# deflect-ca/banjax

Hardware: AMD Instinct MI355X
Metric: log lines/sec matched+rate-limited (node) at 1k rules; HBM GB/s vs peak (higher is better)
Workload: dtype u8

## Files before the change

banjax_amd/_lib.py:

```python
from __future__ import annotations

import ctypes as C
import os

HERE = os.path.dirname(os.path.abspath(__file__))
LIB_PATH = os.environ.get("BJX_LIB_PATH") or os.path.join(HERE, "lib", "libbanjax_gpu.so")

OK = 0
ERR_REGEX, ERR_ARG, ERR_DEVICE, ERR_NOMEM, ERR_TOO_COMPLEX, ERR_CAPACITY, ERR_DECISION = -1, -2, -3, -4, -5, -6, -7
TAIL_STOPPED, ERR_IO = -8, -9
INPUT_DEVICE, COPY_RESULTS, EMIT_BANS, BAN_RECORDS_ONLY, TRIPS_COMPACT, RULE_STATS = 1, 2, 4, 8, 16, 32


class Str(C.Structure):
    _fields_ = [("ptr", C.c_char_p), ("len", C.c_size_t)]


class RuleSpec(C.Structure):
    _fields_ = [("name", Str), ("regex", Str), ("interval_ns", C.c_int64), ("hits_per_interval", C.c_int64),
                ("decision", C.c_int32), ("hosts_to_skip", C.POINTER(Str)), ("n_hosts_to_skip", C.c_size_t)]


class SiteRules(C.Structure):
    _fields_ = [("host", Str), ("rules", C.POINTER(RuleSpec)), ("n_rules", C.c_size_t)]
# ... 207 lines not shown
    L.bjx_finish_batch_trips.argtypes = [vp, vp, C.c_uint64, C.c_uint32, C.POINTER(BatchResult)]
    L.bjx_state_get.restype = C.c_int
    L.bjx_state_get.argtypes = [vp, C.c_char_p, sz, C.c_char_p, sz, C.POINTER(C.c_int64), C.POINTER(C.c_int64)]
    L.bjx_state_len.restype = C.c_int64
    L.bjx_state_len.argtypes = [vp]
    L.bjx_state_stats_get.restype = C.c_int
    L.bjx_state_stats_get.argtypes = [vp, C.c_void_p]
    L.bjx_state_clear.restype = C.c_int
    L.bjx_state_clear.argtypes = [vp]
    L.bjx_state_dump.restype = sz
    L.bjx_state_dump.argtypes = [vp, C.c_char_p, sz]
    L.bjx_debug_rule_match_host.restype = C.c_int
    L.bjx_debug_rule_match_host.argtypes = [vp, sz, C.c_char_p, sz]
    L.bjx_debug_regex_parse.restype = C.c_int
    L.bjx_debug_regex_parse.argtypes = [C.c_char_p, sz, C.c_char_p, sz]
    L.bjx_debug_rule_lead.restype = C.c_int
    L.bjx_debug_rule_lead.argtypes = [vp, sz]
    L.bjx_debug_rule_literal.restype = sz
    L.bjx_debug_rule_literal.argtypes = [vp, sz, C.c_char_p, sz]
    L.bjx_debug_ruleset_literals.restype = sz
    L.bjx_debug_ruleset_literals.argtypes = [vp]
    L.bjx_debug_phase_ms.restype = sz
    L.bjx_debug_phase_ms.argtypes = [vp, C.POINTER(C.c_double), sz]
    L.bjx_debug_kernel_ms.restype = sz
    L.bjx_debug_kernel_ms.argtypes = [vp, C.POINTER(C.c_double), sz]
    L.bjx_debug_scan_stats.restype = sz
    L.bjx_debug_scan_stats.argtypes = [vp, C.POINTER(C.c_uint64), sz]
    L.bjx_debug_set_claim_budget.restype = C.c_int
    L.bjx_debug_set_claim_budget.argtypes = [vp, C.c_uint64]
    L.bjx_debug_set_slot_cache.restype = C.c_int
# ... 113 lines not shown
```

banjax_amd/csrc/engine.hip:

```cpp
#include <hip/hip_runtime.h>
#include <hipcub/hipcub.hpp>

#include <algorithm>
#include <array>
#include <atomic>
#include <cstdio>
#include <cstdlib>
#include <cstring>
#include <map>
#include <set>
#include <tuple>
#include <memory>
#include <mutex>
#include <stdexcept>
#include <string>
#include <unordered_map>
#include <thread>
#include <vector>

#include "../../include/banjax_gpu.h"
#include "bjx_common.h"
#include "engine_types.h"
#include "allow_entry.h"
#include "regex_compiler.h"
#include "bans.h"
#include "snapshot.h"
#include "state_query.h"
#include "state_remove.h"
#include "state_nets.h"
#include "state_trim.h"

using namespace bjx;

namespace {

struct BjxError : std::runtime_error {
// ... 2083 lines not shown
}

__device__ __forceinline__ uint32_t lead_start_seek(const Bind &B, const DevRule &R, const Lines &L, const uint8_t *buf,
                                                    uint64_t n_buf, uint64_t j, uint32_t pos, uint64_t rs, uint32_t rl) {
  const uint32_t st0 = lead_start(B, L, j, pos, rs, rl);
  if ((R.lead & 3u) != 3u || st0 >= rl || B.cfirst || L.cand_meta[j].cnt <= (uint32_t)kCandSlots) return st0;
  const uint32_t back = R.lead_dist ? R.lead_dist + 3u : 0u;
  const uint64_t q = lead_seek(B, R, buf, n_buf, rs + st0 + (st0 ? back : 0u), rs + rl);
  const uint32_t o = (uint32_t)(q - rs);
  return o >= rl ? rl : (o > back && o - back > st0 ? o - back : st0);
}

constexpr uint32_t kDfaLdsEntries = 8192;
constexpr uint32_t kDfaAccelLds = 2048;

__device__ __forceinline__ uint32_t accel_mask(const uint4 v, uint32_t ac) {
  const uint32_t wv[4] = {v.x, v.y, v.z, v.w};
  const uint32_t ne = (ac >> 24) & 3u;
  uint32_t m = 0;
#pragma unroll
  for (int q = 0; q < 4; ++q) {
    uint32_t hb = wv[q] & 0x80808080u;
#pragma unroll
    for (uint32_t k = 0; k < 3; ++k) {
      if (k >= ne) break;
      const uint32_t y = wv[q] ^ (((ac >> (8 * k)) & 0xFFu) * 0x01010101u);
      hb |= ~(((y & 0x7F7F7F7Fu) + 0x7F7F7F7Fu) | y) & 0x80808080u;
    }
    m |= (((hb >> 7) & 1u) | ((hb >> 14) & 2u) | ((hb >> 21) & 4u) | ((hb >> 28) & 8u)) << (4 * q);
  }
  return m;
}

template <bool STAGED>
__device__ __forceinline__ bool dfa_text(const Bind &B, const DevRule &R, const uint16_t *tr, const uint8_t *ac,
                                         const uint32_t *acc, const uint8_t *__restrict__ buf, uint64_t n_buf, uint64_t t0,
                                         uint32_t len, uint32_t st0) {
  const uint32_t ncls = R.ncls;
  uint32_t st = st0;
  uint64_t a = t0 & ~15ull;
  const uint64_t end = t0 + len;
  uint32_t skip = (uint32_t)(t0 - a);
  auto load16 = [&](uint64_t p) -> uint4 {
    if (p + 16 <= n_buf) return *reinterpret_cast<const uint4 *>(buf + p);
    uint32_t w[4];
    for (int k = 0; k < 4; ++k) {
      uint32_t x = 0;
      for (int b = 0; b < 4; ++b) x |= (p + 4 * k + b < n_buf ? (uint32_t)buf[p + 4 * k + b] : 0u) << (8 * b);
      w[k] = x;
    }
    return make_uint4(w[0], w[1], w[2], w[3]);
  };
  uint4 v = a < end ? load16(a) : make_uint4(0, 0, 0, 0);
  while (a < end) {
    const uint32_t aw = acc ? acc[st] : 0u;
    if (aw >> 31) {
      for (;;) {
        uint32_t m = accel_mask(v, aw) & ~((1u << skip) - 1u);
        if (end - a < 16) m &= (1u << (uint32_t)(end - a)) - 1u;
        if (m) { skip = (uint32_t)__ffs(m) - 1; break; }
        a += 16;
        skip = 0;
        if (a >= end) return B.accept_end[R.ae_off + st] != 0;
        v = load16(a);
      }
    }
    const uint4 vn = a + 16 < end ? load16(a + 16) : make_uint4(0, 0, 0, 0);
    const uint32_t wv[4] = {v.x, v.y, v.z, v.w};
    const uint32_t lim = end - a < 16 ? (uint32_t)(end - a) : 16u;
#pragma unroll
    for (uint32_t k = 0; k < 16; ++k) {
      if (k < skip || k >= lim) continue;
      const uint32_t b = (wv[k >> 2] >> (8 * (k & 3))) & 0xFF;
      if (b >= 0x80) {
        const DevRule *Rp = &R;
        uint64_t i = a + k;
        while (i < end) {
          int w;
          const int32_t rune = decode_rune_hd(buf + i, (uint32_t)(end - i), &w);
          uint32_t c;
          if (rune < 0x80) c = ac[rune];
          else {
            const uint32_t *na = B.nonascii + 2 * Rp->na_off;
            uint32_t lo = 0, hi = Rp->n_na;
            while (hi - lo > 1) {
              const uint32_t m = (lo + hi) >> 1;
              if (na[2 * m] <= (uint32_t)rune) lo = m; else hi = m;
            }
            c = na[2 * lo + 1];
          }
          i += (uint32_t)w;
          st = tr[st * ncls + c];
          if (st <= 1) break;
        }
        return B.accept_end[R.ae_off + st] != 0;
      }
      st = tr[st * ncls + ac[b]];
      if (st <= 1) return st == kAccept;
    }
    skip = 0;
    a += 16;
    v = vn;
  }
  return B.accept_end[R.ae_off + st] != 0;
}

__device__ __forceinline__ uint32_t nl_mask16(const uint4 v) {
  return flag_mask16(nl_mask_word(v.x), nl_mask_word(v.y), nl_mask_word(v.z), nl_mask_word(v.w));
}
template <bool STAGED>
__device__ __forceinline__ bool dfa_line(const Bind &B, const DevRule &R, const uint16_t *tr, const uint8_t *ac,
                                         const uint32_t *acc, const uint8_t *__restrict__ buf, uint64_t n_buf, uint64_t t0,
                                         uint32_t st0) {
  const uint32_t ncls = R.ncls;
  uint32_t st = st0;
  uint64_t a = t0 & ~15ull;
  uint32_t skip = (uint32_t)(t0 - a);
  auto load16 = [&](uint64_t p) -> uint4 {
    if (p + 16 <= n_buf) return *reinterpret_cast<const uint4 *>(buf + p);
    uint32_t w[4];
    for (int k = 0; k < 4; ++k) {
      uint32_t x = 0;
      for (int b = 0; b < 4; ++b) x |= (p + 4 * k + b < n_buf ? (uint32_t)buf[p + 4 * k + b] : 0x0Au) << (8 * b);
      w[k] = x;
    }
    return make_uint4(w[0], w[1], w[2], w[3]);
  };
  uint4 v = load16(a);
  for (;;) {
    uint32_t nlm = nl_mask16(v) & ~((1u << skip) - 1u);
    const uint32_t aw = acc ? acc[st] : 0u;
    if ((aw >> 31) && !nlm) {
      for (;;) {
        const uint32_t m = accel_mask(v, aw) & ~((1u << skip) - 1u);
        if (m || nlm) {
          const uint32_t f = (uint32_t)__ffs(m | nlm) - 1;
          skip = f;
          break;
        }
        a += 16;
        skip = 0;
        v = load16(a);
        nlm = nl_mask16(v);
      }
    } else if (aw >> 31) {
      const uint32_t m = (accel_mask(v, aw) | nlm) & ~((1u << skip) - 1u);
      skip = (uint32_t)__ffs(m) - 1;
    }
    const uint32_t lim = nlm ? (uint32_t)__ffs(nlm) - 1 : 16u;
    const uint4 vn = lim == 16u ? load16(a + 16) : make_uint4(0, 0, 0, 0);
    const uint32_t wv[4] = {v.x, v.y, v.z, v.w};
#pragma unroll
    for (uint32_t k = 0; k < 16; ++k) {
      if (k < skip || k >= lim) continue;
      const uint32_t b = (wv[k >> 2] >> (8 * (k & 3))) & 0xFF;
      if (b >= 0x80) {
        uint64_t i = a + k, end = i;
        while (end < n_buf && buf[end] != '\n') ++end;
        while (i < end) {
          int w;
          const int32_t rune = decode_rune_hd(buf + i, (uint32_t)(end - i), &w);
          uint32_t c;
          if (rune < 0x80) c = ac[rune];
          else {
            const uint32_t *na = B.nonascii + 2 * R.na_off;
            uint32_t lo = 0, hi = R.n_na;
            while (hi - lo > 1) {
              const uint32_t m = (lo + hi) >> 1;
              if (na[2 * m] <= (uint32_t)rune) lo = m; else hi = m;
            }
            c = na[2 * lo + 1];
          }
          i += (uint32_t)w;
          st = tr[st * ncls + c];
          if (st <= 1) break;
        }
        return B.accept_end[R.ae_off + st] != 0;
      }
      st = tr[st * ncls + ac[b]];
      if (st <= 1) return st == kAccept;
    }
    if (lim < 16u) return B.accept_end[R.ae_off + st] != 0;
    skip = 0;
    a += 16;
    v = vn;
  }
}

__global__ __launch_bounds__(kBlock) void k_dfa(Bind B, const uint8_t *__restrict__ buf, uint64_t n_buf,
                                                const uint32_t *__restrict__ jkey, const uint32_t *__restrict__ jidx,
                                                const uint32_t *__restrict__ jline, const uint64_t *__restrict__ jrec, uint64_t n,
                                                Lines L) {
  extern __shared__ __attribute__((aligned(16))) uint8_t s_dfa[];
  uint16_t *s_tr = reinterpret_cast<uint16_t *>(s_dfa);
  uint32_t *s_acc = reinterpret_cast<uint32_t *>(s_dfa + ((B.dfa_tr * 2 + 15) & ~15u));
  uint8_t *s_ac = reinterpret_cast<uint8_t *>(s_acc + B.dfa_acc);
  const uint64_t t0 = (uint64_t)blockIdx.x * blockDim.x;
  if ((jkey[t0] & 0xFFFFFF) >= B.n_rules) return;
  const uint64_t t = t0 + threadIdx.x;
  const uint64_t tl = t0 + blockDim.x - 1 < n ? t0 + blockDim.x - 1 : n - 1;
  const uint32_t r0 = jkey[t0] & 0xFFFFFF;
  const DevRule R0 = B.rules[r0];
  const bool uniform = (jkey[tl] & 0xFFFFFF) == r0;
  const bool staged = uniform && (uint32_t)R0.ncls * R0.n_states <= B.dfa_tr;
  if (staged) {
    const uint16_t *g = B.trans + R0.trans_off;
    for (uint32_t i = threadIdx.x; i < (uint32_t)R0.ncls * R0.n_states; i += blockDim.x) s_tr[i] = g[i];
    if (threadIdx.x < 128) s_ac[threadIdx.x] = B.ascii_cls[(size_t)r0 * 128 + threadIdx.x];
    if (R0.n_states <= B.dfa_acc)
      for (uint32_t i = threadIdx.x; i < R0.n_states; i += blockDim.x) s_acc[i] = B.accel[R0.ae_off + i];
  }
  __syncthreads();
  if (t >= n) return;
  const uint32_t key = jkey[t];
  const uint32_t r = key & 0xFFFFFF, pos = key >> 24;
  if (r >= B.n_rules) return;
  const uint32_t slot = jidx[t];
  const uint64_t rec = jrec[slot];
  const uint64_t a = rec & kJobOffMask;
  bool m;
  if (staged) {
    const uint32_t *acc = R0.n_states <= B.dfa_acc ? s_acc : B.accel + R0.ae_off;
    m = dfa_line<true>(B, R0, s_tr, s_ac, acc, buf, n_buf, a, (rec & kJobSkipState) ? R0.skip_state : R0.start);
  } else {
    const DevRule R = B.rules[r];
    m = dfa_line<false>(B, R, B.trans + R.trans_off, B.ascii_cls + (size_t)r * 128, B.accel + R.ae_off, buf, n_buf, a,
                        (rec & kJobSkipState) ? R.skip_state : R.start);
  }
  if (!m) return;
  const uint64_t j = jline[slot];
  atomicOr(reinterpret_cast<unsigned long long *>(&L.mword(j, pos >> 6)), 1ull << (pos & 63));
  atomicAdd(reinterpret_cast<unsigned long long *>(L.counts + j), (1ull << 32) | ((rec & kJobNoCount) ? 0ull : 1ull));
}

__global__ __launch_bounds__(kBlock) void k_dfa_legacy(Bind B, const uint8_t *__restrict__ buf, uint64_t n_buf,
                                                       const uint64_t *__restrict__ nl, const uint32_t *__restrict__ jkey,
                                                       const uint32_t *__restrict__ jidx, const uint32_t *__restrict__ jline,
                                                       uint64_t n, Lines L) {
  __shared__ uint16_t s_tr[kDfaLdsEntries];
  __shared__ uint32_t s_acc[kDfaAccelLds];
  __shared__ uint8_t s_ac[128];
  const uint64_t t0 = (uint64_t)blockIdx.x * blockDim.x;
  const uint64_t t = t0 + threadIdx.x;
  const uint64_t tl = t0 + blockDim.x - 1 < n ? t0 + blockDim.x - 1 : n - 1;
  if ((jkey[tl] & 0xFFFFFF) < B.n_rules) return;
  const uint32_t k0 = jkey[t0] & 0xFFFFFF;
  const uint32_t r0 = k0 >= B.n_rules ? k0 - B.n_rules : k0;
  const DevRule R0 = B.rules[r0];
  const bool uniform = k0 >= B.n_rules && (jkey[tl] & 0xFFFFFF) == k0;
  if (uniform && (R0.flags & kRuleNfa)) return;
  const bool staged = uniform && (uint32_t)R0.ncls * R0.n_states <= kDfaLdsEntries;
  if (staged) {
    const uint16_t *g = B.trans + R0.trans_off;
    for (uint32_t i = threadIdx.x; i < (uint32_t)R0.ncls * R0.n_states; i += blockDim.x) s_tr[i] = g[i];
    if (threadIdx.x < 128) s_ac[threadIdx.x] = B.ascii_cls[(size_t)r0 * 128 + threadIdx.x];
    if (R0.n_states <= kDfaAccelLds)
      for (uint32_t i = threadIdx.x; i < R0.n_states; i += blockDim.x) s_acc[i] = B.accel[R0.ae_off + i];
  }
  __syncthreads();
  if (t >= n) return;
  const uint32_t key = jkey[t];
  const uint32_t rk = key & 0xFFFFFF, pos = key >> 24;
  if (rk < B.n_rules) return;
  const uint32_t r = rk - B.n_rules;
  const uint64_t j = jline[jidx[t]];
  const uint64_t s = j ? nl[j - 1] + 1 : 0;
  const uint64_t rs = s + L.rest_off[j];
  const uint32_t rl = (uint32_t)(nl[j] - rs);
  bool m;
  if (!staged && (B.rules[r].flags & kRuleNfa)) return;
  if ((staged ? R0.equiv : B.rules[r].equiv) && eq_certain(B, L, j, pos, rs)) {
    m = true;
  } else if (staged) {
    const uint32_t sk = R0.skip_len && R0.skip_len <= rl ? R0.skip_len : 0u;
    const uint32_t st0 = (R0.lead & 1u) ? lead_start_seek(B, R0, L, buf, n_buf, j, pos, rs, rl) : 0u;
    const uint32_t *acc = R0.n_states <= kDfaAccelLds ? s_acc : B.accel + R0.ae_off;
    m = st0 ? dfa_text<true>(B, R0, s_tr, s_ac, acc, buf, n_buf, rs + st0, rl - st0, R0.start)
            : dfa_text<true>(B, R0, s_tr, s_ac, acc, buf, n_buf, rs + sk, rl - sk, sk ? R0.skip_state : R0.start);
  } else {
    const DevRule R = B.rules[r];
    const uint32_t sk = R.skip_len && R.skip_len <= rl ? R.skip_len : 0u;
    const uint32_t st0 = (R.lead & 1u) ? lead_start_seek(B, R, L, buf, n_buf, j, pos, rs, rl) : 0u;
    const uint32_t *acc = B.accel + R.ae_off;
    if (st0) m = dfa_text<false>(B, R, B.trans + R.trans_off, B.ascii_cls + (size_t)r * 128, acc, buf, n_buf, rs + st0,
                                 rl - st0, R.start);
    else m = dfa_text<false>(B, R, B.trans + R.trans_off, B.ascii_cls + (size_t)r * 128, acc, buf, n_buf, rs + sk, rl - sk,
                             sk ? R.skip_state : R.start);
  }
  if (!m) return;
  const int32_t hid = L.host_id[j];
  const uint32_t sc = hid >= 0 ? (uint32_t)hid : B.n_hosts;
  const bool no_count = (B.sc_skip[2 * sc + (pos >> 6)] >> (pos & 63)) & 1;
  atomicOr(reinterpret_cast<unsigned long long *>(&L.mword(j, pos >> 6)), 1ull << (pos & 63));
  atomicAdd(reinterpret_cast<unsigned long long *>(L.counts + j), (1ull << 32) | (no_count ? 0ull : 1ull));
}

template <int WT>
__global__ __launch_bounds__(kBlock) void k_nfa(Bind B, uint32_t rule, const uint8_t *__restrict__ buf, uint64_t n_buf,
                                                const uint64_t *__restrict__ nl, const uint32_t *__restrict__ jkey,
                                                const uint32_t *__restrict__ jidx, const uint32_t *__restrict__ jline,
                                                uint64_t j0, uint64_t j1, Lines L) {
  uint64_t *s_b = reinterpret_cast<uint64_t *>(s_dyn);
  const DevRule R = B.rules[rule];
  const uint64_t *g = B.nfa + R.nfa_off;
  const uint32_t total = reinterpret_cast<const uint32_t *>(g)[7];
  for (uint32_t i = threadIdx.x; i < total; i += blockDim.x) s_b[i] = g[i];
  __syncthreads();
  const uint64_t t = j0 + (uint64_t)blockIdx.x * blockDim.x + threadIdx.x;
  if (t >= j1) return;
// ... 1901 lines not shown
      rs->sites.emplace_back(host, std::move(ids));
    }
    if (max_site + n_global >= 65536) { set_err(err, err_len, "more than 65535 rules apply to one host"); return BJX_ERR_TOO_COMPLEX; }
    rs->uid = g_ruleset_uid++;
    *out = rs.release();
    return BJX_OK;
  } catch (const std::exception &e) {
    set_err(err, err_len, e.what());
    return BJX_ERR_NOMEM;
  }
}

extern "C" void bjx_ruleset_release(bjx_ruleset *rs) { delete rs; }
extern "C" size_t bjx_ruleset_num_rules(const bjx_ruleset *rs) { return rs ? rs->rules.size() : 0; }
extern "C" uint64_t bjx_internal_ruleset_serial(const bjx_ruleset *rs) { return rs ? rs->uid : 0; }
extern "C" int bjx_ruleset_rule_info(const bjx_ruleset *rs, size_t i, uint32_t *states, uint32_t *classes, uint32_t *flags) {
  if (!rs || i >= rs->rules.size()) return BJX_ERR_ARG;
  const auto &rx = rs->rules[i].rx;
  if (states) *states = rx.nstates;
  if (classes) *classes = rx.ncls;
  if (flags)
    *flags = rx.flags | ((uint32_t)rx.mode << 8) | (rx.pref_equivalent ? 0x10000u : 0u) | (rx.pref_lead ? 0x20000u : 0u) |
             ((uint32_t)rx.pref.size() << 20);
  return BJX_OK;
}


struct BatchCtx {
  const uint8_t *buf = nullptr;
  uint64_t n_lines = 0, n_res = 0, n_ev = 0;
// ... 393 lines not shown
  std::vector<uint64_t> nfa_blob;
  std::vector<uint32_t> accel;
  std::vector<uint32_t> rule_full;
  std::vector<const std::string *> site_host(rs->rules.size(), nullptr);
  for (auto &st : rs->sites)
    for (uint32_t r : st.second) site_host[r] = &st.first;
  bool any_anchored = false;
  for (size_t i = 0; i < rs->rules.size(); ++i) {
    const auto &r = rs->rules[i];
    DevRule &d = drules[i];
    memset(&d, 0, sizeof d);
    d.trans_off = (uint32_t)trans.size();
    trans.insert(trans.end(), r.rx.trans.begin(), r.rx.trans.end());
    d.ae_off = (uint32_t)ae.size();
    ae.insert(ae.end(), r.rx.accept_end.begin(), r.rx.accept_end.end());
    for (uint32_t st = 0; st < r.rx.accept_end.size(); ++st) {
      uint32_t a = 0;
      if (st > 1 && !(r.rx.flags & kRuleNfa) && !r.rx.trans.empty()) {
        uint32_t esc[3] = {0, 0, 0}, ne = 0;
        bool ok = true;
        for (uint32_t b = 0; b < 128 && ok; ++b)
          if (r.rx.trans[(size_t)st * r.rx.ncls + r.rx.ascii_cls[b]] != st) {
            if (ne == 3) ok = false;
            else esc[ne++] = b;
          }
        if (ok) a = 0x80000000u | (ne << 24) | (esc[2] << 16) | (esc[1] << 8) | esc[0];
      }
      accel.push_back(a);
    }
    d.na_off = (uint32_t)(nonascii.size() / 2);
    for (auto &p : r.rx.nonascii) { nonascii.push_back(p.first); nonascii.push_back(p.second); }
    d.n_na = (uint16_t)r.rx.nonascii.size();
    d.ncls = (uint16_t)r.rx.ncls;
    d.n_states = r.rx.nstates;
    d.start = r.rx.start;
    d.flags = (uint16_t)r.rx.flags;
    memcpy(&ascii[i * 128], r.rx.ascii_cls, 128);
    d.name_id = intern_name(e, r.name);
    d.decision = r.decision;
    d.mode = (uint8_t)r.rx.mode;
    d.equiv = r.rx.pref_equivalent ? 1 : 0;
    auto intern_lit = [&](const PrefLit &pl, bool pref) {
      auto key = std::make_pair(pl.s, pl.ci);
      auto it = lit_ids.find(key);
// ... 1787 lines not shown
  const unsigned long long n_slow = sc4[4], n_slots = sc4[3];
  e->last_jobs = n_jobs;
  e->last_job_rules = B.n_rules;
  e->scan_stats[0] = sc4[0]; e->scan_stats[1] = sc4[1]; e->scan_stats[2] = n_slow; e->scan_stats[3] = B.scan_img_bytes;
  e->scan_stats[4] = n_jobs; e->scan_stats[5] = sc4[2];
  HIP_OK(hipEventRecord(e->evk[2], st));
  if (n_jobs) {
    e->jidx2.ensure(n_slots); e->jkey2.ensure(n_slots);
    {
      uint32_t *ki = e->jkey.p, *ko = e->jkey2.p, *vi = e->jidx.p, *vo = e->jidx2.p;
      const int bits = std::max(1, bit_width(2 * B.n_rules));
      cub_call(e, [&](void *tmp, size_t &bytes) {
        return hipcub::DeviceRadixSort::SortPairs(tmp, bytes, ki, ko, vi, vo, (int)n_slots, 0, bits, st);
      });
    }
    hipLaunchKernelGGL(k_dfa, dim3(grid_for(n_jobs)), dim3(kBlock), B.dfa_lds, st, B, buf, (uint64_t)n, e->jkey2.p,
                       e->jidx2.p, e->jline.p, e->jrec.p, (uint64_t)n_jobs, L);
    hipLaunchKernelGGL(k_dfa_legacy, dim3(grid_for(n_jobs)), dim3(kBlock), 0, st, B, buf, (uint64_t)n, e->nl.p, e->jkey2.p,
                       e->jidx2.p, e->jline.p, (uint64_t)n_jobs, L);
    HIP_OK(hipGetLastError());
    if (B.any_nfa && !e->nfa_rules.empty()) run_nfa_jobs(e, B, buf, n, n_jobs, L);
    static const bool job_stats = getenv("BJX_JOB_STATS") != nullptr;
    if (job_stats) {
      const uint32_t nk = 2 * B.n_rules;
      e->rb_first.ensure(nk); e->rb_last.ensure(nk);
      HIP_OK(hipMemsetAsync(e->rb_first.p, 0, nk * 4ull, st));
      HIP_OK(hipMemsetAsync(e->rb_last.p, 0, nk * 4ull, st));
      hipLaunchKernelGGL(k_rule_bounds, dim3(grid_for(n_jobs)), dim3(kBlock), 0, st, (uint64_t)n_jobs, e->jkey2.p, e->rb_first.p,
                         e->rb_last.p);
      std::vector<uint32_t> f(nk), l(nk);
      HIP_OK(hipMemcpyAsync(f.data(), e->rb_first.p, nk * 4ull, hipMemcpyDeviceToHost, st));
      HIP_OK(hipMemcpyAsync(l.data(), e->rb_last.p, nk * 4ull, hipMemcpyDeviceToHost, st));
      HIP_OK(hipStreamSynchronize(st));
      std::map<std::string, uint64_t> by_rx;
// ... 777 lines not shown
    out->log = out->log_bytes ? e->ban_log.data() : nullptr;
    out->log_off = e->ban_off.data();
    out->log_kind = e->ban_n_trips ? e->ban_kind.data() : nullptr;
    out->ip_bytes = e->ban_ipb.size() ? e->ban_ipb.data() : nullptr;
    out->ip_off = e->ban_ipo.data();
    return BJX_OK;
  });
}

#include "../../include/banjax_gpu_debug.h"

extern "C" int bjx_debug_rule_match_host(const bjx_ruleset *rs, size_t i, const uint8_t *text, size_t n) {
  if (!rs || i >= rs->rules.size() || (n && !text)) return BJX_ERR_ARG;
  return dfa_match_host(rs->rules[i].rx, text, n) ? 1 : 0;
}
extern "C" int bjx_debug_set_dfa_state_cap(uint32_t cap) {
  set_dfa_state_cap(cap);
  std::lock_guard<std::mutex> g(g_rx_mu);
  g_rx_cache.clear();
  return BJX_OK;
}
extern "C" int bjx_debug_force_wide_nfa(int on) {
  set_force_wide_nfa(on != 0);
  std::lock_guard<std::mutex> g(g_rx_mu);
  g_rx_cache.clear();
  return BJX_OK;
}
extern "C" int bjx_debug_set_ip_hash_mask(bjx_engine *e, uint64_t mask) {
  if (!e) return BJX_ERR_ARG;
  std::lock_guard<std::mutex> g(e->mu);
// ... 170 lines not shown
```

include/banjax_gpu_debug.h:

```cpp
#ifndef BANJAX_GPU_DEBUG_H
#define BANJAX_GPU_DEBUG_H
#include <stddef.h>
#include <stdint.h>
#include "banjax_gpu.h"
#ifdef __cplusplus
extern "C" {
#endif
int bjx_debug_rule_match_host(const bjx_ruleset *rs, size_t rule_idx, const uint8_t *text, size_t n);
size_t bjx_debug_rule_literal(const bjx_ruleset *rs, size_t rule_idx, char *out, size_t cap);
size_t bjx_debug_ruleset_literals(const bjx_ruleset *rs);
int bjx_debug_rule_lead(const bjx_ruleset *rs, size_t rule_idx);
int bjx_debug_regex_parse(const char *pattern, size_t len, char *err, size_t err_len);
size_t bjx_debug_phase_ms(bjx_engine *e, double *out, size_t cap);
size_t bjx_debug_kernel_ms(bjx_engine *e, double *out, size_t cap);
size_t bjx_debug_scan_stats(bjx_engine *e, uint64_t *out, size_t cap);
int bjx_debug_set_ip_hash_mask(bjx_engine *e, uint64_t mask);
int bjx_debug_set_claim_budget(bjx_engine *e, uint64_t max_new);
int bjx_debug_set_slot_cache(bjx_engine *e, int on);
int bjx_debug_set_bucket_bits(bjx_engine *e, uint32_t bits);
int bjx_debug_set_trim_grid(bjx_engine *e, uint32_t max_blocks);
int bjx_debug_state_slots(bjx_engine *e, const uint8_t *ip_bytes, const uint32_t *ip_off, const bjx_str *names,
                          size_t n_names, const uint32_t *name_idx, size_t n, int64_t *slots);
int bjx_debug_set_dfa_state_cap(uint32_t cap);
int bjx_debug_force_wide_nfa(int on);
int bjx_debug_set_rule_stats_lds(bjx_engine *e, uint32_t max_rules);
int bjx_debug_rule_stats_path(bjx_engine *e);
int bjx_debug_job_counts(bjx_engine *e, uint32_t *windowed, uint32_t *legacy, size_t n_rules, uint32_t *line_pass_runs);
#ifdef __cplusplus
}
#endif
#endif
```

Baseline: 2.626 billion.

## Rewrite DFA inner loop with pre-scaled staged tables and wave-uniform stepping

```diff
diff --git a/banjax_amd/_lib.py b/banjax_amd/_lib.py
--- a/banjax_amd/_lib.py
+++ b/banjax_amd/_lib.py
@@ -245,6 +245,9 @@
     L.bjx_debug_rule_match_host.argtypes = [vp, sz, C.c_char_p, sz]
     L.bjx_debug_regex_parse.restype = C.c_int
     L.bjx_debug_regex_parse.argtypes = [C.c_char_p, sz, C.c_char_p, sz]
+    if hasattr(L, "bjx_debug_rule_tables"):
+        L.bjx_debug_rule_tables.restype = sz
+        L.bjx_debug_rule_tables.argtypes = [vp, sz, C.c_int, vp, sz]
     L.bjx_debug_rule_lead.restype = C.c_int
     L.bjx_debug_rule_lead.argtypes = [vp, sz]
     L.bjx_debug_rule_literal.restype = sz
diff --git a/banjax_amd/csrc/dfa_step.h b/banjax_amd/csrc/dfa_step.h
--- /dev/null
+++ b/banjax_amd/csrc/dfa_step.h
@@ -0,0 +1,182 @@
+#pragma once
+#include <stdint.h>
+
+#include "bjx_common.h"
+
+namespace bjx {
+
+enum : uint32_t {
+  kDfaNo = 0,
+  kDfaYes = 1,
+  kDfaEnd = 2,
+  kDfaTail = 3,
+};
+struct DfaPos {
+  uint32_t code, st;
+  uint64_t at;
+};
+
+template <class TR, class AC, class ACC>
+struct DfaTabs {
+  TR tr;
+  AC ac;
+  ACC acc;
+  uint32_t ncls;
+  uint32_t inv;
+  uint32_t any_acc;
+};
+
+BJX_HD uint32_t dfa_inv(uint32_t ncls) { return (uint32_t)(0x100000000ull / ncls) + 1u; }
+
+BJX_HD uint32_t dfa_eq_flags(uint32_t v, uint32_t rep) {
+  const uint32_t x = v ^ rep;
+  return ~(((x & 0x7F7F7F7Fu) + 0x7F7F7F7Fu) | x) & 0x80808080u;
+}
+BJX_HD uint32_t dfa_gather16(uint64_t lo, uint64_t hi) {
+#ifdef __HIP_DEVICE_COMPILE__
+  const uint32_t a = __builtin_amdgcn_udot4((uint32_t)(lo >> 32), 0x80402010u,
+                                            __builtin_amdgcn_udot4((uint32_t)lo, 0x08040201u, 0u, false), false);
+  const uint32_t b = __builtin_amdgcn_udot4((uint32_t)(hi >> 32), 0x80402010u,
+                                            __builtin_amdgcn_udot4((uint32_t)hi, 0x08040201u, 0u, false), false);
+  return ((b << 8) | a) >> 7;
+#else
+  uint32_t m = 0;
+  for (uint32_t i = 0; i < 8; ++i) m |= (uint32_t)((lo >> (8 * i + 7)) & 1) << i | (uint32_t)((hi >> (8 * i + 7)) & 1) << (8 + i);
+  return m;
+#endif
+}
+BJX_HD uint32_t dfa_ctz(uint32_t m) { return (uint32_t)__builtin_ctz(m); }
+BJX_HD bool dfa_any(bool x) {
+#ifdef __HIP_DEVICE_COMPILE__
+  return __builtin_amdgcn_ballot_w64(x) != 0;
+#else
+  return x;
+#endif
+}
+BJX_HD void dfa_load16(const uint8_t *p, uint64_t &lo, uint64_t &hi) {
+  __builtin_memcpy(&lo, p, 8);
+  __builtin_memcpy(&hi, p + 8, 8);
+}
+
+BJX_HD uint64_t dfa_esc_flags(uint64_t w, uint32_t aw) {
+  const uint32_t ne = (aw >> 24) & 3u;
+  uint32_t f[2] = {(uint32_t)w & 0x80808080u, (uint32_t)(w >> 32) & 0x80808080u};
+#pragma unroll
+  for (uint32_t k = 0; k < 3; ++k) {
+    if (k >= ne) break;
+    const uint32_t rep = ((aw >> (8 * k)) & 0xFFu) * 0x01010101u;
+    f[0] |= dfa_eq_flags((uint32_t)w, rep);
+    f[1] |= dfa_eq_flags((uint32_t)(w >> 32), rep);
+  }
+  return ((uint64_t)f[1] << 32) | f[0];
+}
+BJX_HD uint64_t dfa_nl_flags(uint64_t w) {
+  return ((uint64_t)dfa_eq_flags((uint32_t)(w >> 32), 0x0A0A0A0Au) << 32) | dfa_eq_flags((uint32_t)w, 0x0A0A0A0Au);
+}
+
+template <bool LINE, bool SCALED, class TR, class AC, class ACC>
+BJX_HD DfaPos dfa_windows(const DfaTabs<TR, AC, ACC> &T, const uint8_t *__restrict__ buf, uint64_t n_buf, uint64_t t0,
+                          uint32_t len, uint32_t st0) {
+  const uint32_t ncls = T.ncls;
+  const uint32_t one = SCALED ? ncls : 1u;
+  uint32_t s = SCALED ? st0 * ncls : st0;
+  auto state = [&](uint32_t x) -> uint32_t { return SCALED ? (uint32_t)(((uint64_t)x * T.inv) >> 32) : x; };
+  const uint64_t r64 = t0 < n_buf ? n_buf - t0 : 0;
+  const uint32_t room = r64 > 0xFFFFFFFFull ? 0xFFFFFFFFu : (uint32_t)r64;
+  uint32_t o = 0;
+  if (!LINE && len == 0) return DfaPos{kDfaEnd, st0, t0};
+  if (room < 16u) return DfaPos{kDfaTail, st0, t0};
+  uint64_t lo, hi;
+  dfa_load16(buf + t0, lo, hi);
+  for (;;) {
+    uint32_t lim;
+    if (LINE) {
+      const uint32_t nlm = dfa_gather16(dfa_nl_flags(lo), dfa_nl_flags(hi));
+      lim = nlm ? dfa_ctz(nlm) : 16u;
+    } else {
+      lim = len - o < 16u ? len - o : 16u;
+    }
+    uint32_t w = 16;
+    if (T.any_acc) {
+      const uint32_t aw = T.acc[state(s)];
+      if (aw >> 31) {
+        uint32_t skip;
+        for (;;) {
+          const bool more = lim == 16u && room - o >= 32u;
+          uint64_t nlo = 0, nhi = 0;
+          if (more) dfa_load16(buf + t0 + o + 16u, nlo, nhi);
+          const uint64_t flo = dfa_esc_flags(lo, aw), fhi = dfa_esc_flags(hi, aw);
+          const uint32_t m = (flo | fhi) ? dfa_gather16(flo, fhi) & ((1u << lim) - 1u) : 0u;
+          if (m) { skip = dfa_ctz(m); break; }
+          if (lim < 16u) return DfaPos{kDfaEnd, state(s), t0 + o + lim};
+          o += 16u;
+          if (!more) return DfaPos{kDfaTail, state(s), t0 + o};
+          lo = nlo; hi = nhi;
+          if (LINE) {
+            const uint32_t nlm = dfa_gather16(dfa_nl_flags(lo), dfa_nl_flags(hi));
+            lim = nlm ? dfa_ctz(nlm) : 16u;
+          } else {
+            lim = len - o < 16u ? len - o : 16u;
+          }
+        }
+        if (skip) {
+          uint32_t sh = 8u * skip;
+          if (sh >= 64u) { lo = hi; hi = 0; sh -= 64u; }
+          if (sh) { lo = (lo >> sh) | (hi << (64u - sh)); hi >>= sh; }
+          o += skip; lim -= skip; w -= skip;
+        }
+      }
+    }
+    uint32_t n = lim;
+    if ((lo | hi) & 0x8080808080808080ull) {
+      const uint32_t hm = dfa_gather16(lo & 0x8080808080808080ull, hi & 0x8080808080808080ull) & ((1u << lim) - 1u);
+      if (hm) n = dfa_ctz(hm);
+    }
+    const bool more = n == w && room - o >= w + 16u;
+    uint64_t nlo = 0, nhi = 0;
+    if (more) dfa_load16(buf + t0 + o + w, nlo, nhi);
+#pragma unroll
+    for (uint32_t k = 0; k < 16; ++k) {
+      if (!dfa_any(k < n)) break;
+      if (k < n) {
+        const uint32_t b = (uint32_t)((k < 8 ? lo >> (8 * k) : hi >> (8 * (k - 8))) & 0xFF);
+        s = T.tr[(SCALED ? s : s * ncls) + T.ac[b]];
+        if (s <= one) return DfaPos{s == one ? kDfaYes : kDfaNo, 0u, 0ull};
+      }
+    }
+    if (n < w) return DfaPos{n == lim ? kDfaEnd : kDfaTail, state(s), t0 + o + n};
+    o += w;
+    if (!more) return DfaPos{kDfaTail, state(s), t0 + o};
+    lo = nlo; hi = nhi;
+  }
+}
+
+template <bool LINE>
+BJX_HD uint32_t dfa_tail(const uint16_t *tr, const uint8_t *ac, const uint32_t *na, uint32_t n_na, uint32_t ncls,
+                         const uint8_t *__restrict__ buf, uint64_t n_buf, uint64_t at, uint64_t end, uint32_t st) {
+  if (LINE) {
+    end = at;
+    while (end < n_buf && buf[end] != '\n') ++end;
+  }
+  uint64_t i = at;
+  while (i < end) {
+    int w;
+    const int32_t rune = decode_rune_hd(buf + i, end - i, &w);
+    uint32_t c;
+    if (rune < 0x80) c = ac[rune];
+    else {
+      uint32_t l = 0, h = n_na;
+      while (h - l > 1) {
+        const uint32_t m = (l + h) >> 1;
+        if (na[2 * m] <= (uint32_t)rune) l = m; else h = m;
+      }
+      c = na[2 * l + 1];
+    }
+    i += (uint32_t)w;
+    st = tr[st * ncls + c];
+    if (st <= 1) break;
+  }
+  return st;
+}
+
+}
diff --git a/banjax_amd/csrc/engine.hip b/banjax_amd/csrc/engine.hip
--- a/banjax_amd/csrc/engine.hip
+++ b/banjax_amd/csrc/engine.hip
@@ -20,6 +20,7 @@
 
 #include "../../include/banjax_gpu.h"
 #include "bjx_common.h"
+#include "dfa_step.h"
 #include "engine_types.h"
 #include "allow_entry.h"
 #include "regex_compiler.h"
@@ -2133,285 +2134,181 @@
 constexpr uint32_t kDfaLdsEntries = 8192;
 constexpr uint32_t kDfaAccelLds = 2048;
 
-__device__ __forceinline__ uint32_t accel_mask(const uint4 v, uint32_t ac) {
-  const uint32_t wv[4] = {v.x, v.y, v.z, v.w};
-  const uint32_t ne = (ac >> 24) & 3u;
-  uint32_t m = 0;
-#pragma unroll
-  for (int q = 0; q < 4; ++q) {
-    uint32_t hb = wv[q] & 0x80808080u;
-#pragma unroll
-    for (uint32_t k = 0; k < 3; ++k) {
-      if (k >= ne) break;
-      const uint32_t y = wv[q] ^ (((ac >> (8 * k)) & 0xFFu) * 0x01010101u);
-      hb |= ~(((y & 0x7F7F7F7Fu) + 0x7F7F7F7Fu) | y) & 0x80808080u;
-    }
-    m |= (((hb >> 7) & 1u) | ((hb >> 14) & 2u) | ((hb >> 21) & 4u) | ((hb >> 28) & 8u)) << (4 * q);
-  }
-  return m;
-}
-
-template <bool STAGED>
-__device__ __forceinline__ bool dfa_text(const Bind &B, const DevRule &R, const uint16_t *tr, const uint8_t *ac,
-                                         const uint32_t *acc, const uint8_t *__restrict__ buf, uint64_t n_buf, uint64_t t0,
-                                         uint32_t len, uint32_t st0) {
-  const uint32_t ncls = R.ncls;
-  uint32_t st = st0;
-  uint64_t a = t0 & ~15ull;
-  const uint64_t end = t0 + len;
-  uint32_t skip = (uint32_t)(t0 - a);
-  auto load16 = [&](uint64_t p) -> uint4 {
-    if (p + 16 <= n_buf) return *reinterpret_cast<const uint4 *>(buf + p);
-    uint32_t w[4];
-    for (int k = 0; k < 4; ++k) {
-      uint32_t x = 0;
-      for (int b = 0; b < 4; ++b) x |= (p + 4 * k + b < n_buf ? (uint32_t)buf[p + 4 * k + b] : 0u) << (8 * b);
-      w[k] = x;
-    }
-    return make_uint4(w[0], w[1], w[2], w[3]);
-  };
-  uint4 v = a < end ? load16(a) : make_uint4(0, 0, 0, 0);
-  while (a < end) {
-    const uint32_t aw = acc ? acc[st] : 0u;
-    if (aw >> 31) {
-      for (;;) {
-        uint32_t m = accel_mask(v, aw) & ~((1u << skip) - 1u);
-        if (end - a < 16) m &= (1u << (uint32_t)(end - a)) - 1u;
-        if (m) { skip = (uint32_t)__ffs(m) - 1; break; }
-        a += 16;
-        skip = 0;
-        if (a >= end) return B.accept_end[R.ae_off + st] != 0;
-        v = load16(a);
-      }
-    }
-    const uint4 vn = a + 16 < end ? load16(a + 16) : make_uint4(0, 0, 0, 0);
-    const uint32_t wv[4] = {v.x, v.y, v.z, v.w};
-    const uint32_t lim = end - a < 16 ? (uint32_t)(end - a) : 16u;
-#pragma unroll
-    for (uint32_t k = 0; k < 16; ++k) {
-      if (k < skip || k >= lim) continue;
-      const uint32_t b = (wv[k >> 2] >> (8 * (k & 3))) & 0xFF;
-      if (b >= 0x80) {
-        const DevRule *Rp = &R;
-        uint64_t i = a + k;
-        while (i < end) {
-          int w;
-          const int32_t rune = decode_rune_hd(buf + i, (uint32_t)(end - i), &w);
-          uint32_t c;
-          if (rune < 0x80) c = ac[rune];
-          else {
-            const uint32_t *na = B.nonascii + 2 * Rp->na_off;
-            uint32_t lo = 0, hi = Rp->n_na;
-            while (hi - lo > 1) {
-              const uint32_t m = (lo + hi) >> 1;
-              if (na[2 * m] <= (uint32_t)rune) lo = m; else hi = m;
-            }
-            c = na[2 * lo + 1];
-          }
-          i += (uint32_t)w;
-          st = tr[st * ncls + c];
-          if (st <= 1) break;
-        }
-        return B.accept_end[R.ae_off + st] != 0;
-      }
-      st = tr[st * ncls + ac[b]];
-      if (st <= 1) return st == kAccept;
-    }
-    skip = 0;
-    a += 16;
-    v = vn;
-  }
-  return B.accept_end[R.ae_off + st] != 0;
-}
-
-__device__ __forceinline__ uint32_t nl_mask16(const uint4 v) {
-  return flag_mask16(nl_mask_word(v.x), nl_mask_word(v.y), nl_mask_word(v.z), nl_mask_word(v.w));
-}
-template <bool STAGED>
-__device__ __forceinline__ bool dfa_line(const Bind &B, const DevRule &R, const uint16_t *tr, const uint8_t *ac,
-                                         const uint32_t *acc, const uint8_t *__restrict__ buf, uint64_t n_buf, uint64_t t0,
-                                         uint32_t st0) {
-  const uint32_t ncls = R.ncls;
-  uint32_t st = st0;
-  uint64_t a = t0 & ~15ull;
-  uint32_t skip = (uint32_t)(t0 - a);
-  auto load16 = [&](uint64_t p) -> uint4 {
-    if (p + 16 <= n_buf) return *reinterpret_cast<const uint4 *>(buf + p);
-    uint32_t w[4];
-    for (int k = 0; k < 4; ++k) {
-      uint32_t x = 0;
-      for (int b = 0; b < 4; ++b) x |= (p + 4 * k + b < n_buf ? (uint32_t)buf[p + 4 * k + b] : 0x0Au) << (8 * b);
-      w[k] = x;
-    }
-    return make_uint4(w[0], w[1], w[2], w[3]);
-  };
-  uint4 v = load16(a);
-  for (;;) {
-    uint32_t nlm = nl_mask16(v) & ~((1u << skip) - 1u);
-    const uint32_t aw = acc ? acc[st] : 0u;
-    if ((aw >> 31) && !nlm) {
-      for (;;) {
-        const uint32_t m = accel_mask(v, aw) & ~((1u << skip) - 1u);
-        if (m || nlm) {
-          const uint32_t f = (uint32_t)__ffs(m | nlm) - 1;
-          skip = f;
-          break;
-        }
-        a += 16;
-        skip = 0;
-        v = load16(a);
-        nlm = nl_mask16(v);
-      }
-    } else if (aw >> 31) {
-      const uint32_t m = (accel_mask(v, aw) | nlm) & ~((1u << skip) - 1u);
-      skip = (uint32_t)__ffs(m) - 1;
-    }
-    const uint32_t lim = nlm ? (uint32_t)__ffs(nlm) - 1 : 16u;
-    const uint4 vn = lim == 16u ? load16(a + 16) : make_uint4(0, 0, 0, 0);
-    const uint32_t wv[4] = {v.x, v.y, v.z, v.w};
-#pragma unroll
-    for (uint32_t k = 0; k < 16; ++k) {
-      if (k < skip || k >= lim) continue;
-      const uint32_t b = (wv[k >> 2] >> (8 * (k & 3))) & 0xFF;
-      if (b >= 0x80) {
-        uint64_t i = a + k, end = i;
-        while (end < n_buf && buf[end] != '\n') ++end;
-        while (i < end) {
-          int w;
-          const int32_t rune = decode_rune_hd(buf + i, (uint32_t)(end - i), &w);
-          uint32_t c;
-          if (rune < 0x80) c = ac[rune];
-          else {
-            const uint32_t *na = B.nonascii + 2 * R.na_off;
-            uint32_t lo = 0, hi = R.n_na;
-            while (hi - lo > 1) {
-              const uint32_t m = (lo + hi) >> 1;
-              if (na[2 * m] <= (uint32_t)rune) lo = m; else hi = m;
-            }
-            c = na[2 * lo + 1];
-          }
-          i += (uint32_t)w;
-          st = tr[st * ncls + c];
-          if (st <= 1) break;
-        }
-        return B.accept_end[R.ae_off + st] != 0;
-      }
-      st = tr[st * ncls + ac[b]];
-      if (st <= 1) return st == kAccept;
-    }
-    if (lim < 16u) return B.accept_end[R.ae_off + st] != 0;
-    skip = 0;
-    a += 16;
-    v = vn;
-  }
-}
-
-__global__ __launch_bounds__(kBlock) void k_dfa(Bind B, const uint8_t *__restrict__ buf, uint64_t n_buf,
+struct DfaArgs {
+  const DevRule *rules;
+  const uint16_t *trans;
+  const uint8_t *accept_end;
+  const uint32_t *accel;
+  const uint8_t *ascii_cls;
+  const uint32_t *nonascii;
+  uint64_t *masks;
+  uint64_t mstride;
+  uint64_t *counts;
+  uint32_t n_rules;
+  uint32_t dfa_tr, dfa_acc;
+};
+static DfaArgs dfa_args(const Bind &B, const Lines &L) {
+  return DfaArgs{B.rules, B.trans, B.accept_end, B.accel, B.ascii_cls, B.nonascii, L.masks, L.mstride, L.counts,
+                 B.n_rules, B.dfa_tr, B.dfa_acc};
+}
+
+template <bool LINE>
+__device__ __forceinline__ bool dfa_finish(const DfaArgs &A, const DevRule &R, uint32_t r, bjx::DfaPos p,
+                                           const uint8_t *__restrict__ buf, uint64_t n_buf, uint64_t end) {
+  if (p.code < bjx::kDfaEnd) return p.code == bjx::kDfaYes;
+  uint32_t st = p.st;
+  if (p.code == bjx::kDfaTail)
+    st = bjx::dfa_tail<LINE>(A.trans + R.trans_off, A.ascii_cls + (size_t)r * 128, A.nonascii + 2 * R.na_off, R.n_na, R.ncls,
+                             buf, n_buf, p.at, end, st);
+  return A.accept_end[R.ae_off + st] != 0;
+}
+
+__device__ __forceinline__ bool dfa_stage(const DfaArgs &A, const DevRule &R0, uint32_t r0, bool acc_fit, uint16_t *s_tr,
+                                          uint32_t *s_acc, uint8_t *s_ac) {
+  const uint16_t *g = A.trans + R0.trans_off;
+  const uint32_t ncls = R0.ncls;
+  for (uint32_t i = threadIdx.x; i < ncls * R0.n_states; i += blockDim.x) s_tr[i] = (uint16_t)(g[i] * ncls);
+  if (threadIdx.x < 128) s_ac[threadIdx.x] = A.ascii_cls[(size_t)r0 * 128 + threadIdx.x];
+  uint32_t any = acc_fit ? 0u : 1u;
+  if (acc_fit)
+    for (uint32_t i = threadIdx.x; i < R0.n_states; i += blockDim.x) {
+      const uint32_t w = A.accel[R0.ae_off + i];
+      s_acc[i] = w;
+      any |= w >> 31;
+    }
+  return __syncthreads_or((int)any) != 0;
+}
+
+__global__ __launch_bounds__(kBlock) void k_dfa(DfaArgs A, const uint8_t *__restrict__ buf, uint64_t n_buf,
                                                 const uint32_t *__restrict__ jkey, const uint32_t *__restrict__ jidx,
-                                                const uint32_t *__restrict__ jline, const uint64_t *__restrict__ jrec, uint64_t n,
-                                                Lines L) {
+                                                const uint32_t *__restrict__ jline, const uint64_t *__restrict__ jrec, uint64_t n) {
   extern __shared__ __attribute__((aligned(16))) uint8_t s_dfa[];
-  uint16_t *s_tr = reinterpret_cast<uint16_t *>(s_dfa);
-  uint32_t *s_acc = reinterpret_cast<uint32_t *>(s_dfa + ((B.dfa_tr * 2 + 15) & ~15u));
-  uint8_t *s_ac = reinterpret_cast<uint8_t *>(s_acc + B.dfa_acc);
+  uint8_t *s_ac = s_dfa;
+  uint16_t *s_tr = reinterpret_cast<uint16_t *>(s_dfa + 128);
+  uint32_t *s_acc = reinterpret_cast<uint32_t *>(s_dfa + 128 + ((A.dfa_tr * 2 + 15) & ~15u));
   const uint64_t t0 = (uint64_t)blockIdx.x * blockDim.x;
-  if ((jkey[t0] & 0xFFFFFF) >= B.n_rules) return;
+  if ((jkey[t0] & 0xFFFFFF) >= A.n_rules) return;
   const uint64_t t = t0 + threadIdx.x;
   const uint64_t tl = t0 + blockDim.x - 1 < n ? t0 + blockDim.x - 1 : n - 1;
   const uint32_t r0 = jkey[t0] & 0xFFFFFF;
-  const DevRule R0 = B.rules[r0];
+  const DevRule R0 = A.rules[r0];
   const bool uniform = (jkey[tl] & 0xFFFFFF) == r0;
-  const bool staged = uniform && (uint32_t)R0.ncls * R0.n_states <= B.dfa_tr;
-  if (staged) {
-    const uint16_t *g = B.trans + R0.trans_off;
-    for (uint32_t i = threadIdx.x; i < (uint32_t)R0.ncls * R0.n_states; i += blockDim.x) s_tr[i] = g[i];
-    if (threadIdx.x < 128) s_ac[threadIdx.x] = B.ascii_cls[(size_t)r0 * 128 + threadIdx.x];
-    if (R0.n_states <= B.dfa_acc)
-      for (uint32_t i = threadIdx.x; i < R0.n_states; i += blockDim.x) s_acc[i] = B.accel[R0.ae_off + i];
-  }
-  __syncthreads();
+  const bool staged = uniform && (uint32_t)R0.ncls * R0.n_states <= A.dfa_tr;
+  const bool acc_fit = R0.n_states <= A.dfa_acc;
+  bool any_acc = true;
+  if (staged) any_acc = dfa_stage(A, R0, r0, acc_fit, s_tr, s_acc, s_ac);
   if (t >= n) return;
   const uint32_t key = jkey[t];
   const uint32_t r = key & 0xFFFFFF, pos = key >> 24;
-  if (r >= B.n_rules) return;
+  if (r >= A.n_rules) return;
   const uint32_t slot = jidx[t];
   const uint64_t rec = jrec[slot];
   const uint64_t a = rec & kJobOffMask;
-  bool m;
+  bjx::DfaPos p;
   if (staged) {
-    const uint32_t *acc = R0.n_states <= B.dfa_acc ? s_acc : B.accel + R0.ae_off;
-    m = dfa_line<true>(B, R0, s_tr, s_ac, acc, buf, n_buf, a, (rec & kJobSkipState) ? R0.skip_state : R0.start);
+    const uint32_t st0 = (rec & kJobSkipState) ? R0.skip_state : R0.start;
+    const uint32_t inv = bjx::dfa_inv(R0.ncls);
+    if (acc_fit) {
+      const bjx::DfaTabs<const uint16_t *, const uint8_t *, const uint32_t *> T{s_tr, s_ac, s_acc, R0.ncls, inv, any_acc};
+      p = bjx::dfa_windows<true, true>(T, buf, n_buf, a, 0u, st0);
+    } else {
+      const bjx::DfaTabs<const uint16_t *, const uint8_t *, const uint32_t *> T{s_tr, s_ac, A.accel + R0.ae_off, R0.ncls, inv, 1u};
+      p = bjx::dfa_windows<true, true>(T, buf, n_buf, a, 0u, st0);
+    }
   } else {
-    const DevRule R = B.rules[r];
-    m = dfa_line<false>(B, R, B.trans + R.trans_off, B.ascii_cls + (size_t)r * 128, B.accel + R.ae_off, buf, n_buf, a,
-                        (rec & kJobSkipState) ? R.skip_state : R.start);
-  }
+    const DevRule R = A.rules[r];
+    const bjx::DfaTabs<const uint16_t *, const uint8_t *, const uint32_t *> T{
+        A.trans + R.trans_off, A.ascii_cls + (size_t)r * 128, A.accel + R.ae_off, R.ncls, 0u, 1u};
+    p = bjx::dfa_windows<true, false>(T, buf, n_buf, a, 0u, (rec & kJobSkipState) ? R.skip_state : R.start);
+  }
+  bool m = p.code == bjx::kDfaYes;
+  if (p.code >= bjx::kDfaEnd) m = dfa_finish<true>(A, A.rules[r], r, p, buf, n_buf, 0);
   if (!m) return;
   const uint64_t j = jline[slot];
-  atomicOr(reinterpret_cast<unsigned long long *>(&L.mword(j, pos >> 6)), 1ull << (pos & 63));
-  atomicAdd(reinterpret_cast<unsigned long long *>(L.counts + j), (1ull << 32) | ((rec & kJobNoCount) ? 0ull : 1ull));
-}
-
-__global__ __launch_bounds__(kBlock) void k_dfa_legacy(Bind B, const uint8_t *__restrict__ buf, uint64_t n_buf,
+  atomicOr(reinterpret_cast<unsigned long long *>(A.masks + (uint64_t)(pos >> 6) * A.mstride + j), 1ull << (pos & 63));
+  atomicAdd(reinterpret_cast<unsigned long long *>(A.counts + j), (1ull << 32) | ((rec & kJobNoCount) ? 0ull : 1ull));
+}
+
+struct DfaLegacyArgs {
+  const uint32_t *global_rules, *site_off, *site_rules, *rule_lits;
+  const uint64_t *sc_skip;
+  const uint8_t *img;
+  ImgLayout il;
+  uint32_t n_hosts, lits_small, cfirst;
+  const uint32_t *rest_off;
+  const int32_t *host_id;
+  const CandMeta *cand_meta;
+  const uint64_t *cand, *cand_first;
+};
+static DfaLegacyArgs dfa_legacy_args(const Bind &B, const Lines &L) {
+  return DfaLegacyArgs{B.global_rules, B.site_off, B.site_rules, B.rule_lits, B.sc_skip, B.img, B.il, B.n_hosts, B.lits_small,
+                       B.cfirst, L.rest_off, L.host_id, L.cand_meta, L.cand, L.cand_first};
+}
+
+__global__ __launch_bounds__(kBlock) void k_dfa_legacy(DfaArgs A, DfaLegacyArgs G, const uint8_t *__restrict__ buf, uint64_t n_buf,
                                                        const uint64_t *__restrict__ nl, const uint32_t *__restrict__ jkey,
                                                        const uint32_t *__restrict__ jidx, const uint32_t *__restrict__ jline,
-                                                       uint64_t n, Lines L) {
+                                                       uint64_t n) {
   __shared__ uint16_t s_tr[kDfaLdsEntries];
   __shared__ uint32_t s_acc[kDfaAccelLds];
   __shared__ uint8_t s_ac[128];
+  Bind B = {};
+  B.rules = A.rules; B.global_rules = G.global_rules; B.site_off = G.site_off; B.site_rules = G.site_rules;
+  B.rule_lits = G.rule_lits; B.img = G.img; B.il = G.il; B.lits_small = G.lits_small; B.cfirst = G.cfirst;
+  Lines L = {};
+  L.rest_off = const_cast<uint32_t *>(G.rest_off); L.host_id = const_cast<int32_t *>(G.host_id);
+  L.cand_meta = const_cast<CandMeta *>(G.cand_meta); L.cand = const_cast<uint64_t *>(G.cand);
+  L.cand_first = const_cast<uint64_t *>(G.cand_first);
   const uint64_t t0 = (uint64_t)blockIdx.x * blockDim.x;
   const uint64_t t = t0 + threadIdx.x;
   const uint64_t tl = t0 + blockDim.x - 1 < n ? t0 + blockDim.x - 1 : n - 1;
-  if ((jkey[tl] & 0xFFFFFF) < B.n_rules) return;
+  if ((jkey[tl] & 0xFFFFFF) < A.n_rules) return;
   const uint32_t k0 = jkey[t0] & 0xFFFFFF;
-  const uint32_t r0 = k0 >= B.n_rules ? k0 - B.n_rules : k0;
-  const DevRule R0 = B.rules[r0];
-  const bool uniform = k0 >= B.n_rules && (jkey[tl] & 0xFFFFFF) == k0;
+  const uint32_t r0 = k0 >= A.n_rules ? k0 - A.n_rules : k0;
+  const DevRule R0 = A.rules[r0];
+  const bool uniform = k0 >= A.n_rules && (jkey[tl] & 0xFFFFFF) == k0;
   if (uniform && (R0.flags & kRuleNfa)) return;
   const bool staged = uniform && (uint32_t)R0.ncls * R0.n_states <= kDfaLdsEntries;
-  if (staged) {
-    const uint16_t *g = B.trans + R0.trans_off;
-    for (uint32_t i = threadIdx.x; i < (uint32_t)R0.ncls * R0.n_states; i += blockDim.x) s_tr[i] = g[i];
-    if (threadIdx.x < 128) s_ac[threadIdx.x] = B.ascii_cls[(size_t)r0 * 128 + threadIdx.x];
-    if (R0.n_states <= kDfaAccelLds)
-      for (uint32_t i = threadIdx.x; i < R0.n_states; i += blockDim.x) s_acc[i] = B.accel[R0.ae_off + i];
-  }
-  __syncthreads();
+  const bool acc_fit = R0.n_states <= kDfaAccelLds;
+  bool any_acc = true;
+  if (staged) any_acc = dfa_stage(A, R0, r0, acc_fit, s_tr, s_acc, s_ac);
   if (t >= n) return;
   const uint32_t key = jkey[t];
   const uint32_t rk = key & 0xFFFFFF, pos = key >> 24;
-  if (rk < B.n_rules) return;
-  const uint32_t r = rk - B.n_rules;
+  if (rk < A.n_rules) return;
+  const uint32_t r = rk - A.n_rules;
   const uint64_t j = jline[jidx[t]];
   const uint64_t s = j ? nl[j - 1] + 1 : 0;
   const uint64_t rs = s + L.rest_off[j];
   const uint32_t rl = (uint32_t)(nl[j] - rs);
   bool m;
-  if (!staged && (B.rules[r].flags & kRuleNfa)) return;
-  if ((staged ? R0.equiv : B.rules[r].equiv) && eq_certain(B, L, j, pos, rs)) {
+  if (!staged && (A.rules[r].flags & kRuleNfa)) return;
+  if ((staged ? R0.equiv : A.rules[r].equiv) && eq_certain(B, L, j, pos, rs)) {
     m = true;
-  } else if (staged) {
-    const uint32_t sk = R0.skip_len && R0.skip_len <= rl ? R0.skip_len : 0u;
-    const uint32_t st0 = (R0.lead & 1u) ? lead_start_seek(B, R0, L, buf, n_buf, j, pos, rs, rl) : 0u;
-    const uint32_t *acc = R0.n_states <= kDfaAccelLds ? s_acc : B.accel + R0.ae_off;
-    m = st0 ? dfa_text<true>(B, R0, s_tr, s_ac, acc, buf, n_buf, rs + st0, rl - st0, R0.start)
-            : dfa_text<true>(B, R0, s_tr, s_ac, acc, buf, n_buf, rs + sk, rl - sk, sk ? R0.skip_state : R0.start);
   } else {
-    const DevRule R = B.rules[r];
+    const DevRule R = staged ? R0 : A.rules[r];
     const uint32_t sk = R.skip_len && R.skip_len <= rl ? R.skip_len : 0u;
-    const uint32_t st0 = (R.lead & 1u) ? lead_start_seek(B, R, L, buf, n_buf, j, pos, rs, rl) : 0u;
-    const uint32_t *acc = B.accel + R.ae_off;
-    if (st0) m = dfa_text<false>(B, R, B.trans + R.trans_off, B.ascii_cls + (size_t)r * 128, acc, buf, n_buf, rs + st0,
-                                 rl - st0, R.start);
-    else m = dfa_text<false>(B, R, B.trans + R.trans_off, B.ascii_cls + (size_t)r * 128, acc, buf, n_buf, rs + sk, rl - sk,
-                             sk ? R.skip_state : R.start);
+    const uint32_t ls = (R.lead & 1u) ? lead_start_seek(B, R, L, buf, n_buf, j, pos, rs, rl) : 0u;
+    const uint32_t off = ls ? ls : sk;
+    const uint32_t st0 = ls || !sk ? R.start : R.skip_state;
+    bjx::DfaPos p;
+    if (staged) {
+      const bjx::DfaTabs<const uint16_t *, const uint8_t *, const uint32_t *> T{
+          s_tr, s_ac, acc_fit ? s_acc : A.accel + R0.ae_off, R0.ncls, bjx::dfa_inv(R0.ncls), any_acc};
+      p = bjx::dfa_windows<false, true>(T, buf, n_buf, rs + off, rl - off, st0);
+    } else {
+      const bjx::DfaTabs<const uint16_t *, const uint8_t *, const uint32_t *> T{
+          A.trans + R.trans_off, A.ascii_cls + (size_t)r * 128, A.accel + R.ae_off, R.ncls, 0u, 1u};
+      p = bjx::dfa_windows<false, false>(T, buf, n_buf, rs + off, rl - off, st0);
+    }
+    m = dfa_finish<false>(A, R, r, p, buf, n_buf, rs + rl);
   }
   if (!m) return;
   const int32_t hid = L.host_id[j];
-  const uint32_t sc = hid >= 0 ? (uint32_t)hid : B.n_hosts;
-  const bool no_count = (B.sc_skip[2 * sc + (pos >> 6)] >> (pos & 63)) & 1;
-  atomicOr(reinterpret_cast<unsigned long long *>(&L.mword(j, pos >> 6)), 1ull << (pos & 63));
-  atomicAdd(reinterpret_cast<unsigned long long *>(L.counts + j), (1ull << 32) | (no_count ? 0ull : 1ull));
+  const uint32_t sc = hid >= 0 ? (uint32_t)hid : G.n_hosts;
+  const bool no_count = (G.sc_skip[2 * sc + (pos >> 6)] >> (pos & 63)) & 1;
+  atomicOr(reinterpret_cast<unsigned long long *>(A.masks + (uint64_t)(pos >> 6) * A.mstride + j), 1ull << (pos & 63));
+  atomicAdd(reinterpret_cast<unsigned long long *>(A.counts + j), (1ull << 32) | (no_count ? 0ull : 1ull));
 }
 
 template <int WT>
@@ -4343,6 +4240,17 @@
 extern "C" void bjx_ruleset_release(bjx_ruleset *rs) { delete rs; }
 extern "C" size_t bjx_ruleset_num_rules(const bjx_ruleset *rs) { return rs ? rs->rules.size() : 0; }
 extern "C" uint64_t bjx_internal_ruleset_serial(const bjx_ruleset *rs) { return rs ? rs->uid : 0; }
+static uint32_t dfa_accel_word(const CompiledRegex &rx, uint32_t st) {
+  if (st <= 1 || (rx.flags & kRuleNfa) || rx.trans.empty()) return 0;
+  uint32_t esc[3] = {0, 0, 0}, ne = 0;
+  for (uint32_t b = 0; b < 128; ++b)
+    if (rx.trans[(size_t)st * rx.ncls + rx.ascii_cls[b]] != st) {
+      if (ne == 3) return 0;
+      esc[ne++] = b;
+    }
+  return 0x80000000u | (ne << 24) | (esc[2] << 16) | (esc[1] << 8) | esc[0];
+}
+
 extern "C" int bjx_ruleset_rule_info(const bjx_ruleset *rs, size_t i, uint32_t *states, uint32_t *classes, uint32_t *flags) {
   if (!rs || i >= rs->rules.size()) return BJX_ERR_ARG;
   const auto &rx = rs->rules[i].rx;
@@ -4766,20 +4674,7 @@
     trans.insert(trans.end(), r.rx.trans.begin(), r.rx.trans.end());
     d.ae_off = (uint32_t)ae.size();
     ae.insert(ae.end(), r.rx.accept_end.begin(), r.rx.accept_end.end());
-    for (uint32_t st = 0; st < r.rx.accept_end.size(); ++st) {
-      uint32_t a = 0;
-      if (st > 1 && !(r.rx.flags & kRuleNfa) && !r.rx.trans.empty()) {
-        uint32_t esc[3] = {0, 0, 0}, ne = 0;
-        bool ok = true;
-        for (uint32_t b = 0; b < 128 && ok; ++b)
-          if (r.rx.trans[(size_t)st * r.rx.ncls + r.rx.ascii_cls[b]] != st) {
-            if (ne == 3) ok = false;
-            else esc[ne++] = b;
-          }
-        if (ok) a = 0x80000000u | (ne << 24) | (esc[2] << 16) | (esc[1] << 8) | esc[0];
-      }
-      accel.push_back(a);
-    }
+    for (uint32_t st = 0; st < r.rx.accept_end.size(); ++st) accel.push_back(dfa_accel_word(r.rx, st));
     d.na_off = (uint32_t)(nonascii.size() / 2);
     for (auto &p : r.rx.nonascii) { nonascii.push_back(p.first); nonascii.push_back(p.second); }
     d.n_na = (uint16_t)r.rx.nonascii.size();
@@ -6597,10 +6492,11 @@
         return hipcub::DeviceRadixSort::SortPairs(tmp, bytes, ki, ko, vi, vo, (int)n_slots, 0, bits, st);
       });
     }
-    hipLaunchKernelGGL(k_dfa, dim3(grid_for(n_jobs)), dim3(kBlock), B.dfa_lds, st, B, buf, (uint64_t)n, e->jkey2.p,
-                       e->jidx2.p, e->jline.p, e->jrec.p, (uint64_t)n_jobs, L);
-    hipLaunchKernelGGL(k_dfa_legacy, dim3(grid_for(n_jobs)), dim3(kBlock), 0, st, B, buf, (uint64_t)n, e->nl.p, e->jkey2.p,
-                       e->jidx2.p, e->jline.p, (uint64_t)n_jobs, L);
+    const DfaArgs DA = dfa_args(B, L);
+    hipLaunchKernelGGL(k_dfa, dim3(grid_for(n_jobs)), dim3(kBlock), B.dfa_lds, st, DA, buf, (uint64_t)n, e->jkey2.p, e->jidx2.p,
+                       e->jline.p, e->jrec.p, (uint64_t)n_jobs);
+    hipLaunchKernelGGL(k_dfa_legacy, dim3(grid_for(n_jobs)), dim3(kBlock), 0, st, DA, dfa_legacy_args(B, L), buf, (uint64_t)n,
+                       e->nl.p, e->jkey2.p, e->jidx2.p, e->jline.p, (uint64_t)n_jobs);
     HIP_OK(hipGetLastError());
     if (B.any_nfa && !e->nfa_rules.empty()) run_nfa_jobs(e, B, buf, n, n_jobs, L);
     static const bool job_stats = getenv("BJX_JOB_STATS") != nullptr;
@@ -7408,6 +7304,35 @@
   if (!rs || i >= rs->rules.size() || (n && !text)) return BJX_ERR_ARG;
   return dfa_match_host(rs->rules[i].rx, text, n) ? 1 : 0;
 }
+extern "C" size_t bjx_debug_rule_tables(const bjx_ruleset *rs, size_t i, int what, void *out, size_t cap) {
+  if (!rs || i >= rs->rules.size()) return 0;
+  const auto &rx = rs->rules[i].rx;
+  if (rx.flags & kRuleNfa) return 0;
+  auto put = [&](const void *p, size_t n, size_t elem) {
+    if (out && cap >= n) memcpy(out, p, n * elem);
+    return n;
+  };
+  switch (what) {
+    case 0: return put(rx.trans.data(), rx.trans.size(), 2);
+    case 1: return put(rx.ascii_cls, 128, 1);
+    case 2: {
+      std::vector<uint32_t> na;
+      for (auto &pr : rx.nonascii) { na.push_back(pr.first); na.push_back(pr.second); }
+      return put(na.data(), na.size(), 4);
+    }
+    case 3: return put(rx.accept_end.data(), rx.accept_end.size(), 1);
+    case 4: {
+      std::vector<uint32_t> acc;
+      for (uint32_t st = 0; st < rx.accept_end.size(); ++st) acc.push_back(dfa_accel_word(rx, st));
+      return put(acc.data(), acc.size(), 4);
+    }
+    case 5: {
+      const uint32_t v[3] = {rx.start, rx.ncls, rx.nstates};
+      return put(v, 3, 4);
+    }
+  }
+  return 0;
+}
 extern "C" int bjx_debug_set_dfa_state_cap(uint32_t cap) {
   set_dfa_state_cap(cap);
   std::lock_guard<std::mutex> g(g_rx_mu);
diff --git a/include/banjax_gpu_debug.h b/include/banjax_gpu_debug.h
--- a/include/banjax_gpu_debug.h
+++ b/include/banjax_gpu_debug.h
@@ -21,6 +21,7 @@
 int bjx_debug_set_trim_grid(bjx_engine *e, uint32_t max_blocks);
 int bjx_debug_state_slots(bjx_engine *e, const uint8_t *ip_bytes, const uint32_t *ip_off, const bjx_str *names,
                           size_t n_names, const uint32_t *name_idx, size_t n, int64_t *slots);
+size_t bjx_debug_rule_tables(const bjx_ruleset *rs, size_t rule_idx, int what, void *out, size_t cap);
 int bjx_debug_set_dfa_state_cap(uint32_t cap);
 int bjx_debug_force_wide_nfa(int on);
 int bjx_debug_set_rule_stats_lds(bjx_engine *e, uint32_t max_rules);
```

After: 2.635 billion, median of 6. About the same (+0.3%).
